# NYXFLOWER/TIP

Measured on AMD Instinct MI355X. Metric: D-D edges aggregated/sec (encoder fwd+bwd), higher is better.
Workload: dtype f32; 1 GPU; TIP-cat full encoder, BioSNAP (645 drugs, 19081 proteins, R=1097), 1xMI355X config; mod=cat, directed_dd_edges=8326508, relations=1097, parallelism=single GPU, launch=hipGraph replay of the captured step, rccl_ranks=0

## Files before the change

### tip_amd/csrc/tipk_drugmix.hip

```cpp
#include "tipk_common.h"
#include "tipk_slabs.h"

namespace {

constexpr int DG_MAX = 64;

struct DgFwdArgs {
    const float* xd; int64_t ld_xd; const float* d_norm;
    const float* h; int64_t ld_h;
    const int32_t* ptr; const int32_t* src; const float* scale;
    const int2* wg;
    const int32_t* order;
    const float* w; int p, q, ne, cat;
    float* out; int64_t ld_out; float* mean;
    int rows;
    const float* basis; const float* root; int n_bases, d_out;
    float* xb;
    float* xroot;
};

constexpr int DG_XMAX = 128;
constexpr int DG_XLD = DG_XMAX + 2;
constexpr int DG_CP = 4;

template <int PL>
__device__ __forceinline__ float dg_row_sum(const float* __restrict__ h, int64_t ld_h, const int32_t* __restrict__ idx, int e0,
                                            int e1, int cc, int lane) {
    constexpr int SLOTS = 64 / PL, STEPS = PL;
    const int s = lane / PL;
    float acc = 0.f;
    int nxt = e0 + lane < e1 ? idx[e0 + lane] : 0;
    for (int b = e0; b < e1; b += 64) {
        const int cur = nxt;
        nxt = b + 64 + lane < e1 ? idx[b + 64 + lane] : 0;
        float v[STEPS];
#pragma unroll
        for (int t = 0; t < STEPS; ++t) {
            const int k = SLOTS * t + s;
            const int row = __shfl(cur, k, 64);
            v[t] = b + k < e1 ? h[(int64_t)row * ld_h + cc] : 0.f;
        }
#pragma unroll
        for (int t = 0; t < STEPS; ++t) acc += v[t];
    }
#pragma unroll
    for (int off = PL; off < 64; off <<= 1) acc += __shfl_xor(acc, off, 64);
    return acc;
}

template <int PL, bool XB>
__global__ __launch_bounds__(1024) void drug_mix_gather_fwd_kernel(DgFwdArgs a) {
    __shared__ float wl[DG_MAX * DG_MAX];
    __shared__ float ml[16][DG_MAX];
    __shared__ float xl[XB ? 16 * DG_XLD : 1];
    __shared__ int rowid[16];
    for (int i = threadIdx.x; i < a.p * a.q; i += 1024) wl[i] = a.w[i];
    if constexpr (XB)
        for (int i = threadIdx.x; i < 16 * DG_XLD; i += 1024) xl[i] = 0.f;
    const int lane = threadIdx.x & 63, wv = threadIdx.x >> 6;
    const int cpart = XB ? (int)(blockIdx.x % DG_CP) : 0;
    const int2 desc = a.wg[XB ? blockIdx.x / DG_CP : blockIdx.x];
    const int nrow = desc.y & 255;
    const int W = (desc.y >> 8) ? (desc.y >> 8) : (nrow == 1 ? 16 : 1);
    const int li = wv / W, sub = wv - li * W;
    const int c = lane % PL;
    const int cc = c < a.p ? c : a.p - 1;
    const bool live = li < nrow;
    int d = 0;
    if (live) d = a.order ? a.order[desc.x + li] : desc.x + li;
    float m = 0.f;
    if (live) {
        int e0 = a.ptr[d], e1 = a.ptr[d + 1];
        if (W > 1) {
            const int per = ((e1 - e0 + W - 1) / W + 63) & ~63;
            e0 = e0 + sub * per;
            e1 = e0 + per < e1 ? e0 + per : e1;
        }
        m = e0 < e1 ? dg_row_sum<PL>(a.h, a.ld_h, a.src, e0, e1, cc, lane) : 0.f;
        if (lane < a.p) ml[wv][lane] = m;
    }
    __syncthreads();
    const int cols = a.cat ? a.ne + a.q : a.ne;
    const bool mine = live && sub == 0;
    if (mine && W > 1) {
        m = 0.f;
        if (lane < a.p)
            for (int k = 0; k < W; ++k) m += ml[wv + k][lane];
    }
    if (!XB && !mine) return;
    if (mine) {
        m *= a.scale[d];
        if (lane < a.p) {
            if (cpart == 0) a.mean[(int64_t)d * a.p + lane] = m;
            ml[wv][lane] = m;
        }
        __builtin_amdgcn_wave_barrier();
        float* o = a.out + (int64_t)d * a.ld_out;
        const float* x = a.xd + (int64_t)d * a.ld_xd;
        for (int col = lane; col < cols; col += 64) {
            float v = 0.f;
            if (col < a.ne) v = a.d_norm ? x[col] / a.d_norm[d] : x[col];
            const int j = a.cat ? col - a.ne : col;
            if (j >= 0 && j < a.q) {
                float t = 0.f;
                for (int k = 0; k < a.p; ++k) t = fmaf(ml[wv][k], wl[k * a.q + j], t);
                v += t;
            }
            if (cpart == 0) o[col] = v;
            if constexpr (XB) xl[li * DG_XLD + col] = v;
        }
        if constexpr (XB)
            if (lane == 0) rowid[li] = d;
    }
    if constexpr (XB) {
        __syncthreads();
        const int m16 = lane & 15, q16 = lane >> 4;
        const int ksteps = cols >> 2;
        const int tpb = a.d_out >> 4;
        const int xb_tiles = a.n_bases * tpb, n_tiles = xb_tiles + tpb;
        const float* xrow = xl + m16 * DG_XLD + q16;
        const int ldw = a.d_out;
        constexpr int TPW = 2;
        constexpr int TS = 16 * DG_CP;
        typedef float f32x4 __attribute__((ext_vector_type(4)));
        for (int t0 = cpart + DG_CP * wv; t0 < n_tiles; t0 += TS * TPW) {
            f32x4 acc[TPW];
            const float* wp[TPW];
#pragma unroll
            for (int i = 0; i < TPW; ++i) {
                acc[i] = f32x4{0.f, 0.f, 0.f, 0.f};
                int tile = t0 + TS * i;
                tile = tile < n_tiles ? tile : n_tiles - 1;
                const bool is_root = tile >= xb_tiles;
                const int b = is_root ? 0 : tile / tpb;
                const int c0 = (is_root ? tile - xb_tiles : tile - b * tpb) << 4;
                wp[i] = (is_root ? a.root : a.basis + (int64_t)b * cols * ldw) + c0 + m16 + q16 * ldw;
            }
            for (int k0 = 0; k0 < ksteps; k0 += 16) {
                float av[16], bw[TPW][16];
#pragma unroll
                for (int i = 0; i < TPW; ++i)
#pragma unroll
                    for (int ks = 0; ks < 16; ++ks) {
                        const int kc = k0 + ks < ksteps ? k0 + ks : ksteps - 1;
                        bw[i][ks] = wp[i][4 * kc * ldw];
                    }
#pragma unroll
                for (int ks = 0; ks < 16; ++ks) {
                    const int kc = k0 + ks < ksteps ? k0 + ks : ksteps - 1;
                    const float v = xrow[4 * kc];
                    av[ks] = k0 + ks < ksteps ? v : 0.f;
                }
#pragma unroll
                for (int ks = 0; ks < 16; ++ks)
#pragma unroll
                    for (int i = 0; i < TPW; ++i)
                        acc[i] = __builtin_amdgcn_mfma_f32_16x16x4f32(av[ks], bw[i][ks], acc[i], 0, 0, 0);
            }
#pragma unroll
            for (int i = 0; i < TPW; ++i) {
                const int tile = t0 + TS * i;
                if (tile < n_tiles) {
                    const bool is_root = tile >= xb_tiles;
                    const int b = is_root ? 0 : tile / tpb;
                    const int c0 = (is_root ? tile - xb_tiles : tile - b * tpb) << 4;
#pragma unroll
                    for (int v = 0; v < 4; ++v) {
                        const int r = 4 * q16 + v;
                        if (r < nrow) {
                            if (is_root) a.xroot[(int64_t)rowid[r] * a.d_out + c0 + m16] = acc[i][v];
                            else a.xb[((int64_t)rowid[r] * a.n_bases + b) * 32 + c0 + m16] = acc[i][v];
                        }
                    }
                }
            }
        }
    }
}

struct DgBwdArgs {
    const float* g; int64_t ld_g;
    const float* d_norm; const float* mean;
    const float* w; int p, q, ne, cat;
    float* g_xd; int64_t ld_gxd;
    float* g_mean;
    float* g_w;
    int rows, n_wg;
    int tp, kg, tile;
};

constexpr int DG_STAGE = 32768;

__global__ __launch_bounds__(1024) void drug_mix_bwd_kernel(DgBwdArgs a) {
    __shared__ float sm[DG_STAGE + 4096];
    const int t = threadIdx.x;
    const int qoff = a.cat ? a.ne : 0;
    if (blockIdx.x == 0) {
        const int hq = a.q / 2;
        const int kgi = t / a.tp, pt = t % a.tp;
        const int pi = pt / hq, pj = pt % hq;
        const int pw = a.p + a.q;
        float s00 = 0.f, s01 = 0.f, s10 = 0.f, s11 = 0.f;
        const int lr = t / pw, lc = t - lr * pw, lrs = 1024 / pw;
        for (int r0 = 0; r0 < a.rows; r0 += a.tile) {
            const int nr = a.rows - r0 < a.tile ? a.rows - r0 : a.tile;
            __syncthreads();
            if (lr < lrs) {
                const float* src = lc < a.p ? a.mean + (int64_t)r0 * a.p + lc : a.g + (int64_t)r0 * a.ld_g + qoff + (lc - a.p);
                const int64_t ld = lc < a.p ? a.p : a.ld_g;
                int r = lr;
                for (; r + 3 * lrs < nr; r += 4 * lrs) {
                    const float v0 = src[(int64_t)r * ld], v1 = src[(int64_t)(r + lrs) * ld];
                    const float v2 = src[(int64_t)(r + 2 * lrs) * ld], v3 = src[(int64_t)(r + 3 * lrs) * ld];
                    sm[r * pw + lc] = v0; sm[(r + lrs) * pw + lc] = v1;
                    sm[(r + 2 * lrs) * pw + lc] = v2; sm[(r + 3 * lrs) * pw + lc] = v3;
                }
                for (; r < nr; r += lrs) sm[r * pw + lc] = src[(int64_t)r * ld];
            }
            __syncthreads();
            if (kgi < a.kg) {
                const float* mrow = sm + 2 * pi;
                const float* grow = sm + a.p + 2 * pj;
                int r = kgi;
                for (; r + 3 * a.kg < nr; r += 4 * a.kg) {
                    const float2 m0 = *reinterpret_cast<const float2*>(mrow + r * pw), g0 = *reinterpret_cast<const float2*>(grow + r * pw);
                    const float2 m1 = *reinterpret_cast<const float2*>(mrow + (r + a.kg) * pw), g1 = *reinterpret_cast<const float2*>(grow + (r + a.kg) * pw);
                    const float2 m2 = *reinterpret_cast<const float2*>(mrow + (r + 2 * a.kg) * pw), g2 = *reinterpret_cast<const float2*>(grow + (r + 2 * a.kg) * pw);
                    const float2 m3 = *reinterpret_cast<const float2*>(mrow + (r + 3 * a.kg) * pw), g3 = *reinterpret_cast<const float2*>(grow + (r + 3 * a.kg) * pw);
                    s00 = fmaf(m0.x, g0.x, s00); s01 = fmaf(m0.x, g0.y, s01); s10 = fmaf(m0.y, g0.x, s10); s11 = fmaf(m0.y, g0.y, s11);
                    s00 = fmaf(m1.x, g1.x, s00); s01 = fmaf(m1.x, g1.y, s01); s10 = fmaf(m1.y, g1.x, s10); s11 = fmaf(m1.y, g1.y, s11);
                    s00 = fmaf(m2.x, g2.x, s00); s01 = fmaf(m2.x, g2.y, s01); s10 = fmaf(m2.y, g2.x, s10); s11 = fmaf(m2.y, g2.y, s11);
                    s00 = fmaf(m3.x, g3.x, s00); s01 = fmaf(m3.x, g3.y, s01); s10 = fmaf(m3.y, g3.x, s10); s11 = fmaf(m3.y, g3.y, s11);
                }
                for (; r < nr; r += a.kg) {
                    const float2 mv = *reinterpret_cast<const float2*>(mrow + r * pw);
                    const float2 gv = *reinterpret_cast<const float2*>(grow + r * pw);
                    s00 = fmaf(mv.x, gv.x, s00); s01 = fmaf(mv.x, gv.y, s01);
                    s10 = fmaf(mv.y, gv.x, s10); s11 = fmaf(mv.y, gv.y, s11);
                }
            }
        }
        float* part = sm + DG_STAGE;
        if (kgi < a.kg) {
            float* sp = part + kgi * (a.p * a.q);
            sp[(2 * pi) * a.q + 2 * pj] = s00; sp[(2 * pi) * a.q + 2 * pj + 1] = s01;
            sp[(2 * pi + 1) * a.q + 2 * pj] = s10; sp[(2 * pi + 1) * a.q + 2 * pj + 1] = s11;
        }
        __syncthreads();
        for (int o = t; o < a.p * a.q; o += 1024) {
            float s = part[o];
            for (int k = 1; k < a.kg; ++k) s += part[k * (a.p * a.q) + o];
            a.g_w[o] = s;
        }
        return;
    }
    const int b = blockIdx.x - 1;
    float* wl = sm;
    if (a.g_mean)
        for (int i = t; i < a.p * a.q; i += 1024) wl[i] = a.w[i];
    if (a.g_xd) {
        const int tot = a.rows * a.ne;
        const int per = (tot + a.n_wg - 1) / a.n_wg;
        const int i1 = (b + 1) * per < tot ? (b + 1) * per : tot;
        for (int i = b * per + t; i < i1; i += 1024) {
            const int r = i / a.ne;
            const int c = i - r * a.ne;
            const float v = a.g[(int64_t)r * a.ld_g + c];
            a.g_xd[(int64_t)r * a.ld_gxd + c] = a.d_norm ? v / a.d_norm[r] : v;
        }
    }
    if (!a.g_mean) return;
    __syncthreads();
    const int tot = a.rows * a.p;
    const int per = (tot + a.n_wg - 1) / a.n_wg;
    const int i1 = (b + 1) * per < tot ? (b + 1) * per : tot;
    for (int i = b * per + t; i < i1; i += 1024) {
        const int r = i / a.p;
        const int c = i - r * a.p;
        const float* gr = a.g + (int64_t)r * a.ld_g + qoff;
        float v = 0.f;
        for (int j = 0; j < a.q; ++j) v = fmaf(gr[j], wl[c * a.q + j], v);
        a.g_mean[i] = v;
    }
}


struct PdBwdArgs {
    DgBwdArgs m;
    const int32_t* tptr; const int32_t* tdst; const float* tw; int n_src;
    const float* agg; int64_t ld_agg; int c1;
    const float* w2; int64_t w2_sk, w2_sn;
    const float* row_scale;
    float* gw; int64_t ld_gw;
    float* dw2; float* db2;
    const int32_t* wg_rows;
    int rows_per_wg;
    int dbg;
};

constexpr int PD_RIDERS = 3;
struct PdRiders {
    int count;
    int first[PD_RIDERS + 1];
    SlabArgs s[PD_RIDERS];
};

constexpr int PD_OFF_WH = 0;
constexpr int PD_OFF_W2 = 4096;
constexpr int PD_OFF_GH = 8192;
constexpr int PD_OFF_AGG = 12288;
constexpr int PD_OFF_TQ = 16384;
constexpr int PD_CHUNK_E = 512;
constexpr int PD_PROD = 16384;
constexpr int PD_OFF_PROD = 20480;
constexpr int PD_OFF_EID = PD_OFF_PROD + PD_PROD;
constexpr int PD_ROWS = 4;
constexpr int PD_WH_WGS = 8;
constexpr int PD_LDS = PD_OFF_EID + 2 * PD_CHUNK_E + 128;
static_assert(PD_LDS >= DG_STAGE + 4096 && PD_LDS * 4 <= 160 * 1024 && PD_LDS >= SLAB_RED_FLOATS, "LDS layout");

template <int PL>
__global__ __launch_bounds__(1024) void pd_stage_bwd_kernel(PdBwdArgs A, PdRiders rd) {
    __shared__ __attribute__((aligned(16))) float sm[PD_LDS];
    if (rd.count > 0 && (int)blockIdx.x >= rd.first[0]) {
        SlabArgs sa = rd.s[0];
        int first = rd.first[0];
#pragma unroll
        for (int q = 1; q < PD_RIDERS; ++q)
            if (q < rd.count && (int)blockIdx.x >= rd.first[q]) { sa = rd.s[q]; first = rd.first[q]; }
        slab_sum_body(sa, (int)blockIdx.x - first, sm);
        return;
    }
    const DgBwdArgs& a = A.m;
    const int t = threadIdx.x;
    const int qoff = a.cat ? a.ne : 0;
    if (blockIdx.x < PD_WH_WGS) {
        if (TIPK_DBG(A.dbg & 1)) return;
        const int share = (a.rows + PD_WH_WGS - 1) / PD_WH_WGS;
        const int ra0 = (int)blockIdx.x * share;
        const int ra1 = ra0 + share < a.rows ? ra0 + share : a.rows;
        const int hq = a.q / 2;
        const int kgi = t / a.tp, pt = t % a.tp;
        const int pi = pt / hq, pj = pt % hq;
        const int pw = a.p + a.q;
        float s00 = 0.f, s01 = 0.f, s10 = 0.f, s11 = 0.f;
        const int lr = t / pw, lc = t - lr * pw, lrs = 1024 / pw;
        for (int r0 = ra0; r0 < ra1; r0 += a.tile) {
            const int nr = ra1 - r0 < a.tile ? ra1 - r0 : a.tile;
            __syncthreads();
            if (lr < lrs) {
                const float* src = lc < a.p ? a.mean + (int64_t)r0 * a.p + lc : a.g + (int64_t)r0 * a.ld_g + qoff + (lc - a.p);
                const int64_t ld = lc < a.p ? a.p : a.ld_g;
                int r = lr;
                for (; r + 3 * lrs < nr; r += 4 * lrs) {
                    const float v0 = src[(int64_t)r * ld], v1 = src[(int64_t)(r + lrs) * ld];
                    const float v2 = src[(int64_t)(r + 2 * lrs) * ld], v3 = src[(int64_t)(r + 3 * lrs) * ld];
                    sm[r * pw + lc] = v0; sm[(r + lrs) * pw + lc] = v1;
                    sm[(r + 2 * lrs) * pw + lc] = v2; sm[(r + 3 * lrs) * pw + lc] = v3;
                }
                for (; r < nr; r += lrs) sm[r * pw + lc] = src[(int64_t)r * ld];
            }
            __syncthreads();
            if (kgi < a.kg) {
                const float* mrow = sm + 2 * pi;
                const float* grow = sm + a.p + 2 * pj;
                int r = kgi;
                for (; r + a.kg < nr; r += 2 * a.kg) {
                    const float2 m0 = *reinterpret_cast<const float2*>(mrow + r * pw), g0 = *reinterpret_cast<const float2*>(grow + r * pw);
                    const float2 m1 = *reinterpret_cast<const float2*>(mrow + (r + a.kg) * pw), g1 = *reinterpret_cast<const float2*>(grow + (r + a.kg) * pw);
                    s00 = fmaf(m0.x, g0.x, s00); s01 = fmaf(m0.x, g0.y, s01); s10 = fmaf(m0.y, g0.x, s10); s11 = fmaf(m0.y, g0.y, s11);
                    s00 = fmaf(m1.x, g1.x, s00); s01 = fmaf(m1.x, g1.y, s01); s10 = fmaf(m1.y, g1.x, s10); s11 = fmaf(m1.y, g1.y, s11);
                }
                for (; r < nr; r += a.kg) {
                    const float2 mv = *reinterpret_cast<const float2*>(mrow + r * pw);
                    const float2 gv = *reinterpret_cast<const float2*>(grow + r * pw);
                    s00 = fmaf(mv.x, gv.x, s00); s01 = fmaf(mv.x, gv.y, s01);
                    s10 = fmaf(mv.y, gv.x, s10); s11 = fmaf(mv.y, gv.y, s11);
                }
            }
        }
        float* part = sm + DG_STAGE;
        if (kgi < a.kg) {
            float* sp = part + kgi * (a.p * a.q);
            sp[(2 * pi) * a.q + 2 * pj] = s00; sp[(2 * pi) * a.q + 2 * pj + 1] = s01;
            sp[(2 * pi + 1) * a.q + 2 * pj] = s10; sp[(2 * pi + 1) * a.q + 2 * pj + 1] = s11;
        }
        __syncthreads();
        float* slab = a.g_w + (int64_t)blockIdx.x * (a.p * a.q);
        for (int o = t; o < a.p * a.q; o += 1024) {
            float s = part[o];
            for (int k = 1; k < a.kg; ++k) s += part[k * (a.p * a.q) + o];
            slab[o] = s;
        }
        return;
    }
    const int b = blockIdx.x - PD_WH_WGS;
    float* wlt = sm + PD_OFF_WH;
    float* w2l = sm + PD_OFF_W2;
    float* gh = sm + PD_OFF_GH;
    float* aggl = sm + PD_OFF_AGG;
    float* tq = sm + PD_OFF_TQ;
    float* prod = sm + PD_OFF_PROD;
    int* eid = reinterpret_cast<int*>(sm + PD_OFF_EID);
    float* ewt = sm + PD_OFF_EID + PD_CHUNK_E;
    int* rptr = reinterpret_cast<int*>(sm + PD_OFF_EID + 2 * PD_CHUNK_E);
    const int p = a.p, q = a.q, c1 = A.c1;
    const int s_first = A.wg_rows[b];
    const int n_mine = A.wg_rows[b + 1] - s_first;
    for (int i = t; i < p * q; i += 1024) wlt[(i % q) * p + i / q] = a.w[i];
    for (int i = t; i < p * c1; i += 1024) w2l[i] = A.w2[(int64_t)(i / c1) * A.w2_sk + (int64_t)(i % c1) * A.w2_sn];
    for (int i = t; i < n_mine * c1; i += 1024) aggl[i] = A.agg[(int64_t)(s_first + i / c1) * A.ld_agg + (i % c1)];
    if (t <= n_mine) rptr[t] = A.tptr[s_first + t];
    if (a.g_xd) {
        const int tot = a.rows * a.ne;
        const int per = (tot + a.n_wg - 1) / a.n_wg;
        const int i1 = (b + 1) * per < tot ? (b + 1) * per : tot;
        for (int i = b * per + t; i < i1; i += 1024) {
            const int r = i / a.ne;
            const int c = i - r * a.ne;
            const float v = a.g[(int64_t)r * a.ld_g + c];
            a.g_xd[(int64_t)r * a.ld_gxd + c] = a.d_norm ? v / a.d_norm[r] : v;
        }
    }
    if (TIPK_DBG(A.dbg & 2)) return;
    __syncthreads();
    const int E0 = rptr[0], E1 = rptr[n_mine];
    constexpr int EPP = 1024 / PL;
    int chunk_e = PD_PROD / q;
    chunk_e = chunk_e < PD_CHUNK_E ? chunk_e : PD_CHUNK_E;
    chunk_e = chunk_e / EPP * EPP;
    const int passes = chunk_e / EPP;
    const int cl = t % PL, el = t / PL;
    const int cq = cl < q ? cl : q - 1;
    float racc[4] = {0.f, 0.f, 0.f, 0.f};
    for (int c0 = E0; c0 < E1; c0 += chunk_e) {
        const int ne_c = E1 - c0 < chunk_e ? E1 - c0 : chunk_e;
        if (t < chunk_e) {
            const bool in = t < ne_c;
            eid[t] = in ? A.tdst[c0 + t] : 0;
            ewt[t] = in ? A.tw[c0 + t] : 0.f;
        }
        __syncthreads();
        if (TIPK_DBG(A.dbg & 16)) return;
        for (int p0 = 0; p0 < passes; p0 += 8) {
            float v[8], w8[8];
#pragma unroll
            for (int u = 0; u < 8; ++u) {
                int e = (p0 + u) * EPP + el;
                e = e < chunk_e ? e : chunk_e - 1;
                w8[u] = ewt[e];
                v[u] = a.g[(int64_t)eid[e] * a.ld_g + qoff + cq];
            }
#pragma unroll
            for (int u = 0; u < 8; ++u) {
                const int e = (p0 + u) * EPP + el;
                if (cl < q && e < chunk_e) prod[e * q + cl] = w8[u] * v[u];
            }
            if ((p0 + 8) * EPP >= ne_c) break;
        }
        __syncthreads();
        if (TIPK_DBG(A.dbg & 32)) return;
#pragma unroll
        for (int k = 0; k < 4; ++k) {
            const int item = t + 1024 * k;
            if (item < n_mine * q) {
                const int r = item / q, c = item - r * q;
                int lo = rptr[r] - c0, hi = rptr[r + 1] - c0;
                lo = lo < 0 ? 0 : lo;
                hi = hi > ne_c ? ne_c : hi;
                float sacc = racc[k];
                int e = lo;
                for (; e + 8 <= hi; e += 8) {
                    float v[8];
#pragma unroll
                    for (int u = 0; u < 8; ++u) v[u] = prod[(e + u) * q + c];
#pragma unroll
                    for (int u = 0; u < 8; ++u) sacc += v[u];
                }
                for (; e < hi; ++e) sacc += prod[e * q + c];
                racc[k] = sacc;
            }
        }
        __syncthreads();
        if (TIPK_DBG(A.dbg & 64)) return;
    }
#pragma unroll
    for (int k = 0; k < 4; ++k) {
        const int item = t + 1024 * k;
        if (item < n_mine * q) tq[item] = racc[k];
    }
    __syncthreads();
    for (int item = t; item < n_mine * p; item += 1024) {
        const int r = item / p, c = item - r * p;
        float v = 0.f;
        for (int j = 0; j < q; ++j) v = fmaf(tq[r * q + j], wlt[j * p + c], v);
        gh[item] = v;
    }
    __syncthreads();
    for (int item = t; item < n_mine * c1; item += 1024) {
        const int r = item / c1, n = item - r * c1;
        const int sr = s_first + r;
        float v = 0.f;
        for (int k = 0; k < p; ++k) v = fmaf(gh[r * p + k], w2l[k * c1 + n], v);
        A.gw[(int64_t)sr * A.ld_gw + n] = A.row_scale ? v * A.row_scale[sr] : v;
    }
    if (TIPK_DBG(A.dbg & 4)) return;
    float* dw = A.dw2 + (int64_t)b * c1 * p;
    for (int o = t; o < c1 * p + p; o += 1024) {
        float sacc = 0.f;
        if (o < c1 * p) {
            const int k = o / p, c = o - k * p;
            for (int r = 0; r < n_mine; ++r) sacc = fmaf(aggl[r * c1 + k], gh[r * p + c], sacc);
            dw[o] = sacc;
        } else {
            const int c = o - c1 * p;
            for (int r = 0; r < n_mine; ++r) sacc += gh[r * p + c];
            A.db2[(int64_t)b * p + c] = sacc;
        }
    }
}

}

extern "C" int tipk_drug_mix_gather_supported(int p, int q) {
    if (p <= 0 || q <= 0 || p > DG_MAX || q > DG_MAX || (p & 1) || (q & 1)) return 0;
    if (p * q / 4 > 1024 || p * q > 4096) return 0;
    return 1;
}

extern "C" int tipk_drug_mix_gather_fwd(const float* xd, int64_t ld_xd, const float* d_norm, const float* h, int64_t ld_h,
                                        const int32_t* ptr, const int32_t* src, const float* scale, const int32_t* wg_desc,
                                        const int32_t* order, int64_t n_wg, const float* w, int p, int q, int64_t rows, int ne, int cat,
                                        float* out, int64_t ld_out, float* mean, tipk_stream_t stream) {
    if (rows < 0 || ne < 0 || !tipk_drug_mix_gather_supported(p, q) || (!cat && q != ne)) return TIPK_EINVAL;
    if (rows == 0) return TIPK_OK;
    if (!xd || !h || !ptr || !src || !scale || !w || !out || !mean || !wg_desc || n_wg <= 0 || rows > 0x7fffffffLL ||
        n_wg > 0x7fffffffLL || (reinterpret_cast<uintptr_t>(wg_desc) & 7))
        return TIPK_EINVAL;
    DgFwdArgs a;
    a.xd = xd; a.ld_xd = ld_xd; a.d_norm = d_norm; a.h = h; a.ld_h = ld_h; a.ptr = ptr; a.src = src; a.scale = scale;
    a.wg = reinterpret_cast<const int2*>(wg_desc); a.order = order;
    a.w = w; a.p = p; a.q = q; a.ne = ne; a.cat = cat; a.out = out; a.ld_out = ld_out; a.mean = mean; a.rows = (int)rows;
    a.basis = nullptr; a.root = nullptr; a.n_bases = 0; a.d_out = 0; a.xb = nullptr; a.xroot = nullptr;
    const dim3 grid((unsigned)n_wg);
    hipStream_t st = (hipStream_t)stream;
    if (p <= 8) hipLaunchKernelGGL((drug_mix_gather_fwd_kernel<8, false>), grid, dim3(1024), 0, st, a);
    else if (p <= 16) hipLaunchKernelGGL((drug_mix_gather_fwd_kernel<16, false>), grid, dim3(1024), 0, st, a);
    else if (p <= 32) hipLaunchKernelGGL((drug_mix_gather_fwd_kernel<32, false>), grid, dim3(1024), 0, st, a);
    else hipLaunchKernelGGL((drug_mix_gather_fwd_kernel<64, false>), grid, dim3(1024), 0, st, a);
    TIPK_RETURN_LAUNCH();
}

extern "C" int tipk_drug_mix_gather_xb_supported(int p, int q, int ne, int cat, int n_bases, int d_out) {
    if (!tipk_drug_mix_gather_supported(p, q) || ne < 0 || (!cat && q != ne)) return 0;
    const int cols = cat ? ne + q : ne;
    if (cols <= 0 || cols > DG_XMAX || (cols & 3)) return 0;
    if (n_bases < 1 || n_bases > 4096 || (d_out != 16 && d_out != 32)) return 0;
    return 1;
}

extern "C" int tipk_drug_mix_gather_xb_fwd(const float* xd, int64_t ld_xd, const float* d_norm, const float* h, int64_t ld_h,
                                           const int32_t* ptr, const int32_t* src, const float* scale, const int32_t* wg_desc,
                                           const int32_t* order, int64_t n_wg, const float* w, int p, int q, int64_t rows, int ne,
                                           int cat, float* out, int64_t ld_out, float* mean, const float* basis, const float* root,
                                           int n_bases, int d_out, float* xb, float* xroot, tipk_stream_t stream) {
    if (rows < 0 || ne < 0) return TIPK_EINVAL;
    if (!tipk_drug_mix_gather_xb_supported(p, q, ne, cat, n_bases, d_out)) return TIPK_EUNSUPPORTED;
    if (rows == 0) return TIPK_OK;
    if (!xd || !h || !ptr || !src || !scale || !w || !out || !mean || !wg_desc || !basis || !root || !xb || !xroot || n_wg <= 0 ||
        rows > 0x7fffffffLL || n_wg > 0x7fffffffLL || (reinterpret_cast<uintptr_t>(wg_desc) & 7))
        return TIPK_EINVAL;
    DgFwdArgs a;
    a.xd = xd; a.ld_xd = ld_xd; a.d_norm = d_norm; a.h = h; a.ld_h = ld_h; a.ptr = ptr; a.src = src; a.scale = scale;
    a.wg = reinterpret_cast<const int2*>(wg_desc); a.order = order;
    a.w = w; a.p = p; a.q = q; a.ne = ne; a.cat = cat; a.out = out; a.ld_out = ld_out; a.mean = mean; a.rows = (int)rows;
    a.basis = basis; a.root = root; a.n_bases = n_bases; a.d_out = d_out; a.xb = xb; a.xroot = xroot;
    if (n_wg * DG_CP > 0x7fffffffLL) return TIPK_EUNSUPPORTED;
    const dim3 grid((unsigned)(n_wg * DG_CP));
    hipStream_t st = (hipStream_t)stream;
    if (p <= 8) hipLaunchKernelGGL((drug_mix_gather_fwd_kernel<8, true>), grid, dim3(1024), 0, st, a);
    else if (p <= 16) hipLaunchKernelGGL((drug_mix_gather_fwd_kernel<16, true>), grid, dim3(1024), 0, st, a);
    else if (p <= 32) hipLaunchKernelGGL((drug_mix_gather_fwd_kernel<32, true>), grid, dim3(1024), 0, st, a);
    else hipLaunchKernelGGL((drug_mix_gather_fwd_kernel<64, true>), grid, dim3(1024), 0, st, a);
    TIPK_RETURN_LAUNCH();
}

extern "C" int tipk_drug_mix_bwd(const float* g, int64_t ld_g, const float* d_norm, const float* mean, const float* w, int p, int q,
                                 int64_t rows, int ne, int cat, float* g_xd, int64_t ld_gxd, float* g_mean, float* g_w,
                                 tipk_stream_t stream) {
    if (rows < 0 || ne < 0 || !tipk_drug_mix_gather_supported(p, q) || (!cat && q != ne)) return TIPK_EINVAL;
    if (rows == 0) return TIPK_OK;
    if (!g || !mean || !w || !g_w || rows * (int64_t)(ne + p + q) > 0x7fffffffLL) return TIPK_EINVAL;
    DgBwdArgs a;
    a.g = g; a.ld_g = ld_g; a.d_norm = d_norm; a.mean = mean; a.w = w; a.p = p; a.q = q; a.ne = ne; a.cat = cat;
    a.g_xd = g_xd; a.ld_gxd = ld_gxd; a.g_mean = g_mean; a.g_w = g_w;
    a.rows = (int)rows;
    a.tp = p * q / 4;
    a.kg = 1024 / a.tp;
    if (a.kg > 4096 / (p * q)) a.kg = 4096 / (p * q);
    if (a.kg > 16) a.kg = 16;
    if (a.kg < 1) a.kg = 1;
    a.tile = DG_STAGE / (p + q);
    int64_t n_wg = tipk_ceil_div(rows * (int64_t)(ne > p ? ne : p), 1024);
    if (n_wg < 1) n_wg = 1;
    if (n_wg > 240) n_wg = 240;
    a.n_wg = (int)n_wg;
    hipLaunchKernelGGL(drug_mix_bwd_kernel, dim3((unsigned)(1 + n_wg)), dim3(1024), 0, (hipStream_t)stream, a);
    TIPK_RETURN_LAUNCH();
}

extern "C" int tipk_pd_stage_bwd_supported(int p, int q, int64_t rows, int c1) {
    if (!tipk_drug_mix_gather_supported(p, q) || rows <= 0) return 0;
    if (c1 <= 0 || c1 > 64 || (int64_t)p * c1 > 4096) return 0;
    return 1;
}

extern "C" int tipk_pd_stage_bwd_wh_slabs(void) { return PD_WH_WGS; }

extern "C" int tipk_pd_stage_bwd_limits(int* max_rows, int* max_edges) {
    if (max_rows) *max_rows = 16 * PD_ROWS;
    if (max_edges) *max_edges = PD_CHUNK_E;
    return TIPK_OK;
}

extern "C" int tipk_pd_stage_bwd(const float* g, int64_t ld_g, const float* d_norm, const float* mean, const float* w, int p, int q,
                                 int64_t rows, int ne, int cat, float* g_xd, int64_t ld_gxd, float* g_w_slabs,
                                 const int32_t* tptr, const int32_t* tdst, const float* tw, int64_t n_src,
                                 const int32_t* wg_rows, int64_t n_row_wg,
                                 const float* agg, int64_t ld_agg, int c1, const float* w2, int64_t w2_sk, int64_t w2_sn,
                                 const float* row_scale, float* gw, int64_t ld_gw, float* dw2_slabs, float* db2_slabs,
                                 tipk_stream_t stream) {
    return tipk_pd_stage_bwd_riders(g, ld_g, d_norm, mean, w, p, q, rows, ne, cat, g_xd, ld_gxd, g_w_slabs, tptr, tdst, tw, n_src, wg_rows,
                                    n_row_wg, agg, ld_agg, c1, w2, w2_sk, w2_sn, row_scale, gw, ld_gw, dw2_slabs, db2_slabs, nullptr, 0,
                                    stream);
}

extern "C" int tipk_pd_stage_bwd_riders(const float* g, int64_t ld_g, const float* d_norm, const float* mean, const float* w, int p,
                                        int q, int64_t rows, int ne, int cat, float* g_xd, int64_t ld_gxd, float* g_w_slabs,
                                        const int32_t* tptr, const int32_t* tdst, const float* tw, int64_t n_src,
                                        const int32_t* wg_rows, int64_t n_row_wg,
                                        const float* agg, int64_t ld_agg, int c1, const float* w2, int64_t w2_sk, int64_t w2_sn,
                                        const float* row_scale, float* gw, int64_t ld_gw, float* dw2_slabs, float* db2_slabs,
                                        const tipk_slab_sum_desc* sums, int32_t n_sums, tipk_stream_t stream) {
    if (n_sums < 0 || n_sums > PD_RIDERS || (n_sums > 0 && !sums)) return TIPK_EINVAL;
    PdRiders rd;
    rd.count = 0;
    int64_t rider_blocks = 0;
    for (int i = 0; i < n_sums; ++i) {
        int rc;
        const int64_t nb = fill_slab_args(sums[i], rd.s[rd.count], &rc);
        if (rc != TIPK_OK) return rc;
        if (nb == 0) continue;
        rd.first[rd.count] = (int)rider_blocks;
        rider_blocks += nb;
        if (rider_blocks > 0x3fffffffLL) return TIPK_EUNSUPPORTED;
        ++rd.count;
    }
    for (int i = rd.count; i <= PD_RIDERS; ++i) rd.first[i] = (int)rider_blocks;
    if (rows < 0 || ne < 0 || n_src < 0) return TIPK_EINVAL;
    if (!tipk_pd_stage_bwd_supported(p, q, rows, c1) || (!cat && q != ne)) return TIPK_EUNSUPPORTED;
    if (!g || !mean || !w || !g_w_slabs || !tptr || !tdst || !tw || !agg || !w2 || !gw || !dw2_slabs || !db2_slabs || n_src == 0 ||
        !wg_rows || n_row_wg <= 0 || n_row_wg > 0x7fffffLL ||
        rows * (int64_t)(ne + p + q) > 0x7fffffffLL || n_src > 0x7fffffffLL)
        return TIPK_EINVAL;
    PdBwdArgs A;
    DgBwdArgs& a = A.m;
    a.g = g; a.ld_g = ld_g; a.d_norm = d_norm; a.mean = mean; a.w = w; a.p = p; a.q = q; a.ne = ne; a.cat = cat;
    a.g_xd = g_xd; a.ld_gxd = ld_gxd; a.g_mean = nullptr; a.g_w = g_w_slabs;
    a.rows = (int)rows;
    a.tp = p * q / 4;
    a.kg = 1024 / a.tp;
    if (a.kg > 4096 / (p * q)) a.kg = 4096 / (p * q);
    if (a.kg > 16) a.kg = 16;
    if (a.kg < 1) a.kg = 1;
    a.tile = DG_STAGE / (p + q);
    A.rows_per_wg = 16 * PD_ROWS;
    A.wg_rows = wg_rows;
    const int64_t n_wg = n_row_wg;
    a.n_wg = (int)n_wg;
    A.tptr = tptr; A.tdst = tdst; A.tw = tw; A.n_src = (int)n_src;
    A.agg = agg; A.ld_agg = ld_agg; A.c1 = c1; A.w2 = w2; A.w2_sk = w2_sk; A.w2_sn = w2_sn; A.row_scale = row_scale;
    A.gw = gw; A.ld_gw = ld_gw; A.dw2 = dw2_slabs; A.db2 = db2_slabs;
    A.dbg = TIPK_DBG(tipk_option(TIPK_OPT_DM_DEBUG));
    const int stage_wgs = PD_WH_WGS + (int)n_wg;
    for (int i = 0; i <= PD_RIDERS; ++i) rd.first[i] += stage_wgs;
    const dim3 grid((unsigned)(stage_wgs + rider_blocks));
    hipStream_t st = (hipStream_t)stream;
    if (q <= 8) hipLaunchKernelGGL(pd_stage_bwd_kernel<8>, grid, dim3(1024), 0, st, A, rd);
    else if (q <= 16) hipLaunchKernelGGL(pd_stage_bwd_kernel<16>, grid, dim3(1024), 0, st, A, rd);
    else if (q <= 32) hipLaunchKernelGGL(pd_stage_bwd_kernel<32>, grid, dim3(1024), 0, st, A, rd);
    else hipLaunchKernelGGL(pd_stage_bwd_kernel<64>, grid, dim3(1024), 0, st, A, rd);
    TIPK_RETURN_LAUNCH();
}
```

Before: 42.53 billion edges/s.

## Hoist drug-mix loads ahead of gather and skip dead second MFMA tile

Issues the per-row scale, d_norm, xd feature loads and the first mixing-weight load before the edge gather, so their latency overlaps the gather instead of following the barrier. Rows are read unconditionally, so dead waves fall back to a valid index rather than branching. The MFMA tile loop now runs only one accumulator when the second tile is out of range, which skips its weight loads and products. It also adds debug-flag switches that can disable parts of the kernel, at some risk of extra register pressure.

```diff
diff --git a/tip_amd/csrc/tipk_drugmix.hip b/tip_amd/csrc/tipk_drugmix.hip
--- a/tip_amd/csrc/tipk_drugmix.hip
+++ b/tip_amd/csrc/tipk_drugmix.hip
@@ -1,3 +1,4 @@
+#include <type_traits>
 #include "tipk_common.h"
 #include "tipk_slabs.h"
 
@@ -17,6 +18,7 @@
     const float* basis; const float* root; int n_bases, d_out;
     float* xb;
     float* xroot;
+    int dbg;
 };
 
 constexpr int DG_XMAX = 128;
@@ -54,11 +56,9 @@
     __shared__ float ml[16][DG_MAX];
     __shared__ float xl[XB ? 16 * DG_XLD : 1];
     __shared__ int rowid[16];
-    for (int i = threadIdx.x; i < a.p * a.q; i += 1024) wl[i] = a.w[i];
-    if constexpr (XB)
-        for (int i = threadIdx.x; i < 16 * DG_XLD; i += 1024) xl[i] = 0.f;
     const int lane = threadIdx.x & 63, wv = threadIdx.x >> 6;
     const int cpart = XB ? (int)(blockIdx.x % DG_CP) : 0;
+    const int cols = a.cat ? a.ne + a.q : a.ne;
     const int2 desc = a.wg[XB ? blockIdx.x / DG_CP : blockIdx.x];
     const int nrow = desc.y & 255;
     const int W = (desc.y >> 8) ? (desc.y >> 8) : (nrow == 1 ? 16 : 1);
@@ -66,21 +66,57 @@
     const int c = lane % PL;
     const int cc = c < a.p ? c : a.p - 1;
     const bool live = li < nrow;
-    int d = 0;
-    if (live) d = a.order ? a.order[desc.x + li] : desc.x + li;
+    const int slot = live ? desc.x + li : 0;
+    const int ordv = *(a.order ? a.order + slot : a.ptr);
+    const int d = a.order ? ordv : slot;
+    typedef float f32x4 __attribute__((ext_vector_type(4)));
+    constexpr int TPW = 2;
+    constexpr int TS = 16 * DG_CP;
+    const int m16 = lane & 15, q16 = lane >> 4;
+    const int ksteps = cols >> 2;
+    const int tpb = a.d_out >> 4;
+    const int xb_tiles = a.n_bases * tpb, n_tiles = xb_tiles + tpb;
+    const int ldw = a.d_out;
+    auto tile_weights = [&](int tile) {
+        tile = tile < n_tiles ? tile : n_tiles - 1;
+        const bool is_root = tile >= xb_tiles;
+        const int b = is_root ? 0 : tile / tpb;
+        const int c0 = (is_root ? tile - xb_tiles : tile - b * tpb) << 4;
+        return (is_root ? a.root : a.basis + (int64_t)b * cols * ldw) + c0 + m16 + q16 * ldw;
+    };
+    const int t_first = cpart + DG_CP * __builtin_amdgcn_readfirstlane(wv);
+    const float w_first = (int)threadIdx.x < a.p * a.q ? a.w[threadIdx.x] : 0.f;
+    if constexpr (XB)
+        for (int i = threadIdx.x; i < 16 * DG_XLD; i += 1024) xl[i] = 0.f;
+    float sc = 1.f, dn = 1.f, xv[2] = {0.f, 0.f};
+    if constexpr (XB) {
+        if (!TIPK_DBG(a.dbg & 2)) {
+            sc = a.scale[d];
+            dn = *(a.d_norm ? a.d_norm + d : a.scale + d);
+            const float* x = a.xd + (int64_t)d * a.ld_xd;
+#pragma unroll
+            for (int it = 0; it < 2; ++it) {
+                const int col = lane + 64 * it;
+                xv[it] = *(a.ne > 0 ? x + (col < a.ne ? col : a.ne - 1) : a.scale + d);
+            }
+        }
+    }
     float m = 0.f;
+    int e0 = a.ptr[d], e1 = a.ptr[d + 1];
     if (live) {
-        int e0 = a.ptr[d], e1 = a.ptr[d + 1];
-        if (W > 1) {
-            const int per = ((e1 - e0 + W - 1) / W + 63) & ~63;
-            e0 = e0 + sub * per;
-            e1 = e0 + per < e1 ? e0 + per : e1;
-        }
-        m = e0 < e1 ? dg_row_sum<PL>(a.h, a.ld_h, a.src, e0, e1, cc, lane) : 0.f;
+        if (!TIPK_DBG(a.dbg & 1)) {
+            if (W > 1) {
+                const int per = ((e1 - e0 + W - 1) / W + 63) & ~63;
+                e0 = e0 + sub * per;
+                e1 = e0 + per < e1 ? e0 + per : e1;
+            }
+            m = e0 < e1 ? dg_row_sum<PL>(a.h, a.ld_h, a.src, e0, e1, cc, lane) : 0.f;
+        }
         if (lane < a.p) ml[wv][lane] = m;
     }
+    if ((int)threadIdx.x < a.p * a.q) wl[threadIdx.x] = w_first;
+    for (int i = threadIdx.x + 1024; i < a.p * a.q; i += 1024) wl[i] = a.w[i];
     __syncthreads();
-    const int cols = a.cat ? a.ne + a.q : a.ne;
     const bool mine = live && sub == 0;
     if (mine && W > 1) {
         m = 0.f;
@@ -89,17 +125,20 @@
     }
     if (!XB && !mine) return;
     if (mine) {
-        m *= a.scale[d];
+        if constexpr (!XB) {
+            sc = a.scale[d];
+            if (a.d_norm) dn = a.d_norm[d];
+        }
+        m *= sc;
         if (lane < a.p) {
             if (cpart == 0) a.mean[(int64_t)d * a.p + lane] = m;
             ml[wv][lane] = m;
         }
         __builtin_amdgcn_wave_barrier();
         float* o = a.out + (int64_t)d * a.ld_out;
-        const float* x = a.xd + (int64_t)d * a.ld_xd;
-        for (int col = lane; col < cols; col += 64) {
+        auto mix = [&](int col, float xc) {
             float v = 0.f;
-            if (col < a.ne) v = a.d_norm ? x[col] / a.d_norm[d] : x[col];
+            if (col < a.ne) v = a.d_norm ? xc / dn : xc;
             const int j = a.cat ? col - a.ne : col;
             if (j >= 0 && j < a.q) {
                 float t = 0.f;
@@ -108,54 +147,60 @@
             }
             if (cpart == 0) o[col] = v;
             if constexpr (XB) xl[li * DG_XLD + col] = v;
-        }
-        if constexpr (XB)
+        };
+        if constexpr (XB) {
+#pragma unroll
+            for (int it = 0; it < 2; ++it)
+                if (lane + 64 * it < cols) mix(lane + 64 * it, xv[it]);
             if (lane == 0) rowid[li] = d;
+        } else {
+            const float* x = a.xd + (int64_t)d * a.ld_xd;
+            for (int col = lane; col < cols; col += 64) mix(col, col < a.ne ? x[col] : 0.f);
+        }
     }
     if constexpr (XB) {
         __syncthreads();
-        const int m16 = lane & 15, q16 = lane >> 4;
-        const int ksteps = cols >> 2;
-        const int tpb = a.d_out >> 4;
-        const int xb_tiles = a.n_bases * tpb, n_tiles = xb_tiles + tpb;
         const float* xrow = xl + m16 * DG_XLD + q16;
-        const int ldw = a.d_out;
-        constexpr int TPW = 2;
-        constexpr int TS = 16 * DG_CP;
-        typedef float f32x4 __attribute__((ext_vector_type(4)));
-        for (int t0 = cpart + DG_CP * wv; t0 < n_tiles; t0 += TS * TPW) {
+        for (int t0 = t_first; t0 < n_tiles; t0 += TS * TPW) {
+            const bool two = t0 + TS < n_tiles;
             f32x4 acc[TPW];
             const float* wp[TPW];
 #pragma unroll
             for (int i = 0; i < TPW; ++i) {
                 acc[i] = f32x4{0.f, 0.f, 0.f, 0.f};
-                int tile = t0 + TS * i;
-                tile = tile < n_tiles ? tile : n_tiles - 1;
-                const bool is_root = tile >= xb_tiles;
-                const int b = is_root ? 0 : tile / tpb;
-                const int c0 = (is_root ? tile - xb_tiles : tile - b * tpb) << 4;
-                wp[i] = (is_root ? a.root : a.basis + (int64_t)b * cols * ldw) + c0 + m16 + q16 * ldw;
+                wp[i] = tile_weights(t0 + TS * i);
             }
             for (int k0 = 0; k0 < ksteps; k0 += 16) {
                 float av[16], bw[TPW][16];
 #pragma unroll
-                for (int i = 0; i < TPW; ++i)
+                for (int i = 0; i < TPW; ++i) {
+                    if (i > 0 && !two) continue;
 #pragma unroll
                     for (int ks = 0; ks < 16; ++ks) {
                         const int kc = k0 + ks < ksteps ? k0 + ks : ksteps - 1;
-                        bw[i][ks] = wp[i][4 * kc * ldw];
+                        bw[i][ks] = TIPK_DBG(a.dbg & 4) ? 1.f : wp[i][4 * kc * ldw];
                     }
+                }
 #pragma unroll
                 for (int ks = 0; ks < 16; ++ks) {
                     const int kc = k0 + ks < ksteps ? k0 + ks : ksteps - 1;
                     const float v = xrow[4 * kc];
                     av[ks] = k0 + ks < ksteps ? v : 0.f;
                 }
-#pragma unroll
-                for (int ks = 0; ks < 16; ++ks)
-#pragma unroll
-                    for (int i = 0; i < TPW; ++i)
-                        acc[i] = __builtin_amdgcn_mfma_f32_16x16x4f32(av[ks], bw[i][ks], acc[i], 0, 0, 0);
+                auto products = [&](auto nt) __attribute__((always_inline)) {
+#pragma unroll
+                    for (int ks = 0; ks < 16; ++ks)
+#pragma unroll
+                        for (int i = 0; i < decltype(nt)::value; ++i) {
+                            if (TIPK_DBG(a.dbg & 8)) {
+                                asm volatile("" : : "v"(av[ks]), "v"(bw[i][ks]));
+                                continue;
+                            }
+                            acc[i] = __builtin_amdgcn_mfma_f32_16x16x4f32(av[ks], bw[i][ks], acc[i], 0, 0, 0);
+                        }
+                };
+                if (two) products(std::integral_constant<int, TPW>());
+                else products(std::integral_constant<int, 1>());
             }
 #pragma unroll
             for (int i = 0; i < TPW; ++i) {
@@ -541,7 +586,7 @@
     a.xd = xd; a.ld_xd = ld_xd; a.d_norm = d_norm; a.h = h; a.ld_h = ld_h; a.ptr = ptr; a.src = src; a.scale = scale;
     a.wg = reinterpret_cast<const int2*>(wg_desc); a.order = order;
     a.w = w; a.p = p; a.q = q; a.ne = ne; a.cat = cat; a.out = out; a.ld_out = ld_out; a.mean = mean; a.rows = (int)rows;
-    a.basis = nullptr; a.root = nullptr; a.n_bases = 0; a.d_out = 0; a.xb = nullptr; a.xroot = nullptr;
+    a.basis = nullptr; a.root = nullptr; a.n_bases = 0; a.d_out = 0; a.xb = nullptr; a.xroot = nullptr; a.dbg = 0;
     const dim3 grid((unsigned)n_wg);
     hipStream_t st = (hipStream_t)stream;
     if (p <= 8) hipLaunchKernelGGL((drug_mix_gather_fwd_kernel<8, false>), grid, dim3(1024), 0, st, a);
@@ -575,6 +620,7 @@
     a.wg = reinterpret_cast<const int2*>(wg_desc); a.order = order;
     a.w = w; a.p = p; a.q = q; a.ne = ne; a.cat = cat; a.out = out; a.ld_out = ld_out; a.mean = mean; a.rows = (int)rows;
     a.basis = basis; a.root = root; a.n_bases = n_bases; a.d_out = d_out; a.xb = xb; a.xroot = xroot;
+    a.dbg = TIPK_DBG(tipk_option(TIPK_OPT_DP_DEBUG));
     if (n_wg * DG_CP > 0x7fffffffLL) return TIPK_EUNSUPPORTED;
     const dim3 grid((unsigned)(n_wg * DG_CP));
     hipStream_t st = (hipStream_t)stream;
```

Result: no change. 42.82 billion edges/s (median of 6 runs) (+0.7%).
